# Mictronics/multi-sdr-gps-sim

Measured on NVIDIA H100. Metric: IQ Msamples/s, higher is better.
Workload: dtype f64 NCO / int32 accumulate / int8 out

## Files before the change

### include/gpsb200.h

```cpp
#ifndef GPSB200_H
#define GPSB200_H

#include <stdbool.h>
#include <stddef.h>
#include <stdint.h>

#ifdef __cplusplus
extern "C" {
#endif

#define GPSB200_SAMPLERATE        3000000
#define GPSB200_BLOCK_SAMPLES     300000
#define GPSB200_BLOCK_ELEMS       600000
#define GPSB200_MAX_CHAN          32
#define GPSB200_NAV_WORDS         60
#define GPSB200_CA_LEN            1023
#define GPSB200_SC08              1
#define GPSB200_SC16              2
#define GPSB200_HACKRF_BUFFER     262144

enum {
    GPSB200_OK = 0,
    GPSB200_ERR_ARG = -1,
    GPSB200_ERR_CUDA = -2,
// ... 63 lines not shown
    int32_t reset_inside[GPSB200_MAX_CHAN];
    double first_phase[GPSB200_MAX_CHAN];
    double value[GPSB200_MAX_CHAN];
} gpsb200_slice_link_t;
int gpsb200_slice_prepare(gpsb200_ctx_t *ctx, const gpsb200_chan_t *chans, int nblk, int nchan, int sample_size,
                          void *dst_device, void *dst_host, void *stream, gpsb200_slice_link_t *link);
int gpsb200_slice_wait(gpsb200_ctx_t *ctx);
int gpsb200_slice_probe(gpsb200_ctx_t *ctx, const int32_t *prn_in, const double *phase_guess_in, int eager);
int gpsb200_slice_finish(gpsb200_ctx_t *ctx, const int32_t *prn_in, const double *phase_in, int32_t *prn_out,
                         double *phase_out, gpsb200_stats_t *stats);
typedef void (*gpsb200_handoff_fn)(void *user, const int32_t *prn_out, const double *phase_out);
int gpsb200_slice_finish_cb(gpsb200_ctx_t *ctx, const int32_t *prn_in, const double *phase_in, int32_t *prn_out,
                            double *phase_out, gpsb200_stats_t *stats, gpsb200_handoff_fn handoff, void *user);
int gpsb200_slice_link_host(const gpsb200_chan_t *chans, int nblk, int nchan, gpsb200_slice_link_t *link);
int gpsb200_link_apply(const gpsb200_slice_link_t *link, int nchan, const int32_t *prn_in, const double *phase_in,
                       int32_t *prn_out, double *phase_out);

int gpsb200_debug_corrupt_chain(gpsb200_ctx_t *ctx, int on);

int gpsb200_debug_run_checkpoints(gpsb200_ctx_t *ctx, int nblk, int nchan, void *out);

int gpsb200_debug_block_probes(gpsb200_ctx_t *ctx, int nblk, int nchan, void *probes_out, double *seg_out,
                               double *guess_out);

int gpsb200_debug_synth_shape(gpsb200_ctx_t *ctx, int nblk, int nchan, int sample_size, const char **kernel,
                              int *ctas_per_block, int *runs_per_cta);

const char *gpsb200_synth_kernel_name(const gpsb200_ctx_t *ctx, int nchan);

int gpsb200_replay_device(gpsb200_ctx_t *ctx, void *dst_device, void *stream, int kernel_mask);

double gpsb200_carrier_advance(double carr_phase, double f_carr, int64_t nsamples);

int gpsb200_carrier_chain(const gpsb200_chan_t *chans, int nblk, int nchan, const double *phase_in,
                          double *phase_out, int threads);

int gpsb200_carrier_chain_device(gpsb200_ctx_t *ctx, const gpsb200_chan_t *chans, int nblk, int nchan,
                                 const double *phase_in, double *phase_out);

int gpsb200_carrier_probe_fixup(double start, double guess, double f_carr, int64_t nsamples, double *end_out);

int gpsb200_span_chain_host(const double *f_carr, int nblk, double start_true, double start_guess, double *starts_out);

int gpsb200_checkpoint_segments_host(double start_true, double start_guess, double f_carr, int run_samples,
                                     double *starts_out, int *nseg_out);

int gpsb200_carrier_probe_host(double guess, double f_carr, int64_t nsamples, int run_samples, int mode, void *probe_out,
                               double *seg_out);

int gpsb200_lanes_model_block(const gpsb200_chan_t *chans, int nchan, const uint32_t *nav, int run_samples, int force,
                              int16_t *iq, double *carr_out, int64_t *counters, uint32_t *signs);

int gpsb200_lanes_window_band_host(const uint32_t *steps, const uint32_t *bases, int64_t n, uint8_t *out);

int gpsb200_codegen(int prn, uint8_t ca[GPSB200_CA_LEN]);

#define GPSB200_ACQ_MAX_MS    100
#define GPSB200_ACQ_MAX_BINS  1024
#define GPSB200_ACQ_CODE_SAMPLES 3000
typedef struct gpsb200_acq_config {
    int64_t s0;
    int32_t ms;
    int32_t nprn;
    int32_t prn[32];
    double f_lo_hz;
    double step_hz;
    int32_t nbins;
    int32_t reserved;
} gpsb200_acq_config_t;
typedef struct gpsb200_acq_result {
    int32_t prn;
    int32_t bin;
    int32_t delay;
    int32_t reserved;
    double doppler_hz;
    double delay_chips;
    uint64_t p1, p2;
    double ratio;
} gpsb200_acq_result_t;
int gpsb200_acquire(gpsb200_ctx_t *ctx, const void *iq, int64_t nsamples, int sample_size, const gpsb200_acq_config_t *cfg,
                    gpsb200_acq_result_t *res, uint64_t *grid);
int gpsb200_acquire_device(gpsb200_ctx_t *ctx, const void *iq_device, int64_t nsamples, int sample_size,
                           const gpsb200_acq_config_t *cfg, gpsb200_acq_result_t *res, uint64_t *grid, void *stream);
int gpsb200_acquire_windows(gpsb200_ctx_t *ctx, const void *iq, int64_t nsamples, int sample_size,
                            const gpsb200_acq_config_t *cfg, const double *f_lo_prn, gpsb200_acq_result_t *res,
                            uint64_t *grid);
int gpsb200_debug_acq_split(gpsb200_ctx_t *ctx, int force, int nprn, int nbins);
int gpsb200_acquire_windows_device(gpsb200_ctx_t *ctx, const void *iq_device, int64_t nsamples, int sample_size,
                                   const gpsb200_acq_config_t *cfg, const double *f_lo_prn, gpsb200_acq_result_t *res,
                                   uint64_t *grid, void *stream);

#define GPSB200_TRK_CODE_STEP_NOM 1464583848u
#define GPSB200_TRK_CODE_STEP_MIN 1464095816u
#define GPSB200_TRK_CODE_STEP_MAX 1465072205u
#define GPSB200_TRK_FLL_EPOCHS    200
#define GPSB200_TRK_MAX_CHAN      32
typedef struct gpsb200_track_state {
    int32_t prn;
    int32_t epochs;
    int64_t sample;
    uint64_t code_phase;
    int64_t carr_freq;
    uint32_t carr_phase;
    int32_t carr_step;
    uint32_t code_step;
    int32_t prev_i, prev_q;
// ... 427 lines not shown
```

### multi-sdr-gps-sim_b200/__init__.py

```python
from .api import (
    BLOCK_ELEMS, BLOCK_SAMPLES, SC08, SC16, Chan, Config, Context, GpsB200Error, Stats,
    bind_numa, carrier_advance, span_chain_host, lanes_model_block, lanes_window_band, link_apply, slice_link_host, SliceLink, carrier_chain, codegen, scenario, lib, lib_path, CHAN_DTYPE,
    ScenarioConfig, LiveScenario, SteerState, parse_steer, KEYS, ERR_END, almanac_read, ALMANAC_RECORD_DTYPE, checkpoint_segments_host, RUN_CKPT_DTYPE,
    carrier_probe_host, CARRIER_PROBE_DTYPE, AcqConfig, ACQ_RESULT_DTYPE, ACQ_CODE_SAMPLES, acq_window_samples,
    TRACK_STATE_DTYPE, TRACK_EPOCH_DTYPE, NAV_BIT_DTYPE, NAV_WORD_DTYPE, NAV_SYNC_DTYPE, track_start, nav_decode, nav_word_check,
    nav_parity, EPHEMERIS_DTYPE, IONO_DTYPE, PVT_CHAN_DTYPE, PVT_CONFIG_DTYPE, FIX_DTYPE, FIX_OK, FIX_FEW,
    FIX_NO_CONVERGENCE, PVT_MAX_ITER, nav_words_of_frame, nav_ephemeris, nav_time_anchor, pvt_config,
    RAIM_CONFIG_DTYPE, RAIM_DTYPE, RAIM_PASS, RAIM_EXCLUDED, RAIM_ALERT, RAIM_UNAVAILABLE, RAIM_MAX_DOF,
    RAIM_MAX_EXCLUDE, raim_config, raim_thresholds, ARAIM_CONFIG_DTYPE, ARAIM_DTYPE, araim_config, araim_kfa,
    COARSE_CONFIG_DTYPE, COARSE_DTYPE, FIX_AMBIGUOUS, coarse_config, rinex_ephemeris,
    SEARCH_CONFIG_DTYPE, SEARCH_DTYPE, SEARCH_NODES, search_config, search_nodes,
    SKY_DTYPE, nav_almanac, almanac_predict,
    SNAPSHOT_CONFIG_DTYPE, SNAPSHOT_DTYPE, SNAP_OK, SNAP_WEAK, SNAP_NO_CONVERGENCE, SNAP_ITERATIONS, SNAP_MAX_ITER,
    snapshot_config, SNAP_BATCH_SCRATCH, snapshot_batch_pass,
    COLLECTIVE_CONFIG_DTYPE, COLLECTIVE_DTYPE, CD_SCORE_DTYPE, CD_CELL_DTYPE, CD_OK, CD_FEW, CD_AMBIGUOUS, CD_MAX_HYP,
    CD_MIN_USED, CD_Q_SHIFT, CD_Q_CAP, CD_AMBIGUOUS_PCT, collective_config,
)
from .synthetic import synthetic_chans
from . import sharding
```

### multi-sdr-gps-sim_b200/api.py

```python
import ctypes as C
import os

import numpy as np

BLOCK_SAMPLES = 300000
BLOCK_ELEMS = 600000
SC08, SC16 = 1, 2

_HERE = os.path.dirname(os.path.abspath(__file__))


def lib_path():
    return os.path.join(_HERE, "libgpsb200.so")


class GpsB200Error(RuntimeError):
    def __init__(self, code, msg):
        super().__init__("gpsb200 error %d: %s" % (code, msg))
        self.code = code


class Chan(C.Structure):
    _fields_ = [("prn", C.c_int32), ("iword", C.c_int32), ("ibit", C.c_int32), ("icode", C.c_int32),
                ("nav_frame", C.c_int32), ("reserved", C.c_int32),
# ... 320 lines not shown
    if rc:
        raise GpsB200Error(rc, "gpsb200_nav_almanac")
    return rec, int(wna.value)


SKY_DTYPE = np.dtype([("prn", "<i4"), ("valid", "<i4"), ("el_deg", "<f8"), ("az_deg", "<f8"), ("range_m", "<f8"),
                      ("doppler_hz", "<f8")])
assert SKY_DTYPE.itemsize == 40


def almanac_predict(rec, week, sow, x_a):
    r = np.ascontiguousarray(rec, dtype=ALMANAC_RECORD_DTYPE)
    assert r.size == 32
    x = np.ascontiguousarray(x_a, dtype=np.float64).reshape(3)
    out = np.zeros(32, SKY_DTYPE)
    rc = lib().gpsb200_almanac_predict(r.ctypes.data, int(week), float(sow), x.ctypes.data, out.ctypes.data)
    if rc:
        raise GpsB200Error(rc, "gpsb200_almanac_predict")
    return out


def nav_time_anchor(words, sync):
    w = np.ascontiguousarray(words, dtype=NAV_WORD_DTYPE)
    sy = np.array(sync, dtype=NAV_SYNC_DTYPE).reshape(1)
    ep, ms = C.c_int32(0), C.c_int64(0)
    rc = lib().gpsb200_nav_time_anchor(w.ctypes.data if w.size else None, w.size, sy.ctypes.data, C.byref(ep), C.byref(ms))
    if rc:
        raise GpsB200Error(rc, "gpsb200_nav_time_anchor")
    return int(ep.value), int(ms.value)


def pvt_config(s0, step, nfix, iono=None):
    c = np.zeros(1, PVT_CONFIG_DTYPE)[0]
    c["s0"], c["step"], c["nfix"] = int(s0), int(step), int(nfix)
    if iono is not None:
        c["iono"] = 1
        c["alpha"], c["beta"] = np.asarray(iono[0], np.float64), np.asarray(iono[1], np.float64)
    return c


HANDOFF_FN = C.CFUNCTYPE(None, C.c_void_p, C.POINTER(C.c_int32), C.POINTER(C.c_double))

_lib = None

EXPORTS = ["gpsb200_create", "gpsb200_destroy", "gpsb200_last_error", "gpsb200_version", "gpsb200_set_nav",
           "gpsb200_synth_blocks", "gpsb200_synth_blocks_scatter", "gpsb200_synth_blocks_device", "gpsb200_replay_device",
           "gpsb200_carrier_advance", "gpsb200_carrier_chain", "gpsb200_carrier_chain_device", "gpsb200_carrier_probe_fixup",
           "gpsb200_codegen", "gpsb200_acquire", "gpsb200_acquire_device", "gpsb200_acquire_windows",
           "gpsb200_acquire_windows_device", "gpsb200_debug_acq_split", "gpsb200_nav_almanac", "gpsb200_almanac_predict", "gpsb200_track_start",
           "gpsb200_track",
           "gpsb200_track_device", "gpsb200_nav_decode", "gpsb200_nav_word_check", "gpsb200_nav_parity",
           "gpsb200_nav_ephemeris", "gpsb200_nav_time_anchor", "gpsb200_pvt", "gpsb200_pvt_replay",
           "gpsb200_pvt_raim", "gpsb200_raim_thresholds", "gpsb200_pvt_araim", "gpsb200_araim_kfa", "gpsb200_pvt_coarse", "gpsb200_pvt_search", "gpsb200_search_nodes", "gpsb200_snapshot_measure", "gpsb200_snapshot_measure_device", "gpsb200_snapshot_batch", "gpsb200_snapshot_batch_device", "gpsb200_pvt_snapshot", "gpsb200_pvt_snapshot_search", "gpsb200_collective", "gpsb200_collective_device", "gpsb200_rinex_ephemeris", "gpsb200_bind_numa", "gpsb200_span_chain_host", "gpsb200_lanes_model_block",
           "gpsb200_lanes_window_band_host", "gpsb200_slice_prepare", "gpsb200_slice_probe",
           "gpsb200_slice_finish", "gpsb200_slice_finish_cb", "gpsb200_slice_wait", "gpsb200_link_apply", "gpsb200_slice_link_host", "gpsb200_debug_corrupt_chain", "gpsb200_synth_kernel_name",
           "gpsb200_debug_run_checkpoints", "gpsb200_checkpoint_segments_host",
           "gpsb200_carrier_probe_host", "gpsb200_debug_block_probes", "gpsb200_debug_synth_shape",
           "gpsb200_scenario_create", "gpsb200_scenario_destroy", "gpsb200_scenario_error",
           "gpsb200_scenario_blocks", "gpsb200_scenario_channels", "gpsb200_scenario_nav_frames",
           "gpsb200_scenario_chans", "gpsb200_scenario_nav", "gpsb200_scenario_almanac_date", "gpsb200_almanac_read",
           "gpsb200_scenario_open", "gpsb200_scenario_advance", "gpsb200_scenario_frame", "gpsb200_scenario_key",
           "gpsb200_scenario_steer_state", "gpsb200_scenario_open_now", "gpsb200_scenario_create_now",
           "gpsb200_scenario_start_date", "gpsb200_scenario_start_time",
           "fifo_create", "fifo_destroy", "fifo_wait_next", "fifo_wait_full", "fifo_halt", "fifo_acquire",
           "fifo_enqueue", "fifo_dequeue", "fifo_release", "fifo_set_compat_drop",
           "gpsb200_iqfile_start", "gpsb200_iqfile_stop", "gpsb200_fifo_push", "gpsb200_fifo_push_flush"]


def lib():
    global _lib
    if _lib is None:
        if not os.path.exists(lib_path()):
            raise GpsB200Error(-2, "libgpsb200.so not built (run __graft_entry__.build()); there is no CPU fallback")
        L = C.CDLL(lib_path())
        L.gpsb200_create.argtypes = [C.POINTER(Config), C.POINTER(C.c_void_p)]
        L.gpsb200_destroy.argtypes = [C.c_void_p]
        L.gpsb200_last_error.argtypes = [C.c_void_p]
        L.gpsb200_last_error.restype = C.c_char_p
        L.gpsb200_version.restype = C.c_char_p
        L.gpsb200_set_nav.argtypes = [C.c_void_p, C.c_int, C.c_int, C.c_void_p]
        L.gpsb200_synth_blocks.argtypes = [C.c_void_p, C.c_void_p, C.c_int, C.c_int, C.c_int, C.c_void_p,
                                           C.c_void_p, C.POINTER(Stats)]
        L.gpsb200_synth_blocks_scatter.argtypes = [C.c_void_p, C.c_void_p, C.c_int, C.c_int, C.c_int, C.c_void_p,
                                                   C.c_void_p, C.POINTER(Stats)]
        L.gpsb200_synth_blocks_device.argtypes = [C.c_void_p, C.c_void_p, C.c_int, C.c_int, C.c_int, C.c_void_p,
                                                  C.c_void_p, C.c_void_p, C.POINTER(Stats)]
        L.gpsb200_replay_device.argtypes = [C.c_void_p, C.c_void_p, C.c_void_p, C.c_int]
        L.gpsb200_carrier_advance.argtypes = [C.c_double, C.c_double, C.c_int64]
        L.gpsb200_carrier_advance.restype = C.c_double
        L.gpsb200_codegen.argtypes = [C.c_int, C.c_void_p]
        L.gpsb200_scenario_create.argtypes = [C.POINTER(ScenarioConfig), C.POINTER(C.c_void_p)]
        L.gpsb200_scenario_destroy.argtypes = [C.c_void_p]
        L.gpsb200_scenario_error.argtypes = [C.c_void_p]
        L.gpsb200_scenario_error.restype = C.c_char_p
        for fn in ("blocks", "channels", "nav_frames"):
            getattr(L, "gpsb200_scenario_" + fn).argtypes = [C.c_void_p]
        L.gpsb200_scenario_chans.argtypes = [C.c_void_p]
        L.gpsb200_scenario_chans.restype = C.c_void_p
        L.gpsb200_scenario_nav.argtypes = [C.c_void_p]
        L.gpsb200_scenario_nav.restype = C.c_void_p
        L.gpsb200_scenario_almanac_date.argtypes = [C.c_void_p]
        L.gpsb200_scenario_almanac_date.restype = C.c_char_p
        L.gpsb200_almanac_read.argtypes = [C.c_char_p, C.c_void_p, C.POINTER(C.c_int32)]
        L.gpsb200_scenario_open.argtypes = [C.POINTER(ScenarioConfig), C.POINTER(C.c_void_p)]
        L.gpsb200_scenario_open_now.argtypes = [C.POINTER(ScenarioConfig), C.POINTER(C.c_void_p)]
        L.gpsb200_scenario_create_now.argtypes = [C.POINTER(ScenarioConfig), C.POINTER(C.c_void_p)]
        L.gpsb200_scenario_start_date.argtypes = [C.c_void_p]
# ... 91 lines not shown
    ca = np.zeros(1023, np.uint8)
    rc = lib().gpsb200_codegen(prn, ca.ctypes.data)
    if rc:
        raise GpsB200Error(rc, "gpsb200_codegen(%d)" % prn)
    return ca


def carrier_advance(phase, f_carr, nsamples):
    return lib().gpsb200_carrier_advance(float(phase), float(f_carr), int(nsamples))


def carrier_chain(chans, phase_in=None, threads=16):
    a = np.ascontiguousarray(chans, dtype=CHAN_DTYPE)
    nblk, nchan = a.shape
    out = np.zeros(nchan, np.float64)
    pin = None if phase_in is None else np.ascontiguousarray(phase_in, dtype=np.float64)
    rc = lib().gpsb200_carrier_chain(a.ctypes.data, nblk, nchan, None if pin is None else pin.ctypes.data,
                                     out.ctypes.data, threads)
    if rc:
        raise GpsB200Error(rc, "gpsb200_carrier_chain")
    return out


def lanes_model_block(chans_row, nav_frame, run_samples=2400, force=0, want_signs=False):
    a = np.ascontiguousarray(chans_row, dtype=CHAN_DTYPE)
    nv = np.ascontiguousarray(nav_frame, dtype=np.uint32)
    iq = np.zeros(BLOCK_ELEMS, np.int16)
    co = np.zeros(a.size, np.float64)
    cnt = np.zeros(4, np.int64)
    signs = np.zeros((a.size, BLOCK_SAMPLES // 96, 3), np.uint32) if want_signs else None
    L = lib()
    L.gpsb200_lanes_model_block.argtypes = [C.c_void_p, C.c_int, C.c_void_p, C.c_int, C.c_int, C.c_void_p, C.c_void_p, C.c_void_p,
                                            C.c_void_p]
    rc = L.gpsb200_lanes_model_block(a.ctypes.data, a.size, nv.ctypes.data, run_samples, force, iq.ctypes.data, co.ctypes.data,
                                     cnt.ctypes.data, None if signs is None else signs.ctypes.data)
    if rc:
        raise GpsB200Error(rc, "gpsb200_lanes_model_block")
    return (iq, co, cnt, signs) if want_signs else (iq, co, cnt)


def lanes_window_band(steps, bases):
    st, bs = np.broadcast_arrays(np.asarray(steps, np.uint32), np.asarray(bases, np.uint32))
    st = np.ascontiguousarray(st.ravel())
    bs = np.ascontiguousarray(bs.ravel())
    out = np.zeros(st.size, np.uint8)
    L = lib()
    L.gpsb200_lanes_window_band_host.argtypes = [C.c_void_p, C.c_void_p, C.c_int64, C.c_void_p]
    rc = L.gpsb200_lanes_window_band_host(st.ctypes.data, bs.ctypes.data, st.size, out.ctypes.data)
    if rc:
        raise GpsB200Error(rc, "gpsb200_lanes_window_band_host")
    return out.astype(bool)


def span_chain_host(f_carr, start_true, start_guess):
    f = np.ascontiguousarray(f_carr, dtype=np.float64)
    out = np.zeros(f.size + 1)
    rc = lib().gpsb200_span_chain_host(f.ctypes.data, f.size, float(start_true), float(start_guess), out.ctypes.data)
    if rc < 0:
        raise GpsB200Error(rc, "gpsb200_span_chain_host")
    return out if rc == 1 else None


def checkpoint_segments_host(start_true, start_guess, f_carr, run_samples=2400):
    out = np.zeros(8)
    nseg = C.c_int(0)
    rc = lib().gpsb200_checkpoint_segments_host(float(start_true), float(start_guess), float(f_carr), int(run_samples),
                                            out.ctypes.data, C.byref(nseg))
    if rc < 0:
        raise GpsB200Error(rc, "gpsb200_checkpoint_segments_host")
    return rc == 1, out[:nseg.value]


def carrier_probe_host(guess, f_carr, nsamples=BLOCK_SAMPLES, run_samples=2400, mode=1):
    probe = np.zeros(1, CARRIER_PROBE_DTYPE)
    seg = np.zeros((2, 7))
    rc = lib().gpsb200_carrier_probe_host(float(guess), float(f_carr), int(nsamples), int(run_samples), int(mode),
                                          probe.ctypes.data, seg.ctypes.data)
    if rc:
        raise GpsB200Error(rc, "gpsb200_carrier_probe_host")
    return probe[0], seg


def slice_link_host(chans):
    a = np.ascontiguousarray(chans, dtype=CHAN_DTYPE)
    link = SliceLink()
    rc = lib().gpsb200_slice_link_host(a.ctypes.data, a.shape[0], a.shape[1], C.byref(link))
    if rc:
        raise GpsB200Error(rc, "gpsb200_slice_link_host")
    return link


def link_apply(link, nchan, prn_in=None, phase_in=None):
    pi = None if prn_in is None else np.ascontiguousarray(prn_in, dtype=np.int32)
    xi = None if phase_in is None else np.ascontiguousarray(phase_in, dtype=np.float64)
    po, xo = np.zeros(nchan, np.int32), np.zeros(nchan, np.float64)
    rc = lib().gpsb200_link_apply(C.byref(link), nchan, None if pi is None else pi.ctypes.data,
                                  None if xi is None else xi.ctypes.data, po.ctypes.data, xo.ctypes.data)
    if rc:
        raise GpsB200Error(rc, "gpsb200_link_apply")
    return po, xo


def almanac_read(path):
    rec = np.zeros(32, ALMANAC_RECORD_DTYPE)
    valid = C.c_int32(0)
    rc = lib().gpsb200_almanac_read(os.fsencode(path), rec.ctypes.data, C.byref(valid))
# ... 549 lines not shown
```

### multi-sdr-gps-sim_b200/csrc/synth_kernels.h

```cpp
#pragma once
#include <cuda_runtime.h>
#include <stdint.h>

namespace gpsb200 {

constexpr int kBlockSamples = 300000;
constexpr int kNavWords = 60;
constexpr int kChipWords = 33;
constexpr int kAtabRows = 513;

struct BlockChanDev {
    double c_carr;
    double c_code;
    double gain;
    double carr_in;
    double code0;
    int32_t prn;
    uint32_t nav0;
    int32_t frame;
    int32_t pad[3];
};
static_assert(sizeof(BlockChanDev) == 64, "BlockChanDev layout");

struct RunCkpt {
    double x;
    double y;
    uint32_t nav;
    uint32_t pad;
};
static_assert(sizeof(RunCkpt) == 24, "RunCkpt layout");

struct CarrierProbe;
struct SpanBlockState;

struct SpanRes {
    double start;
    double shift;
    int32_t variant;
    int32_t mode;
};
static_assert(sizeof(SpanRes) == 24, "SpanRes layout");

struct SynthArgs {
    const BlockChanDev *bc;
    const double *carr0;
    const double *guess;
    CarrierProbe *probe;
    CarrierProbe *probe_host;
    double *seg;
    CarrierProbe *span_sum;
    SpanBlockState *spec;
    const SpanRes *span_res;
    int span_blocks, nspan;
    RunCkpt *ck;
    const uint32_t *nav;
    int nav_stride;
    const uint32_t *chipbits;
    int32_t *atab;
    double *carr_end;
    double *last_end_host;
    int *chain_errors;
    void *out;
    int nblk, nchan, nruns, run_samples, runs_per_cta, ctas_per_block, iq16;
    int lanes;
};

cudaError_t launch_tables(const SynthArgs &a, cudaStream_t s);
cudaError_t launch_probe(const SynthArgs &a, cudaStream_t s);
cudaError_t launch_chain(const SynthArgs &a, cudaStream_t s);
cudaError_t launch_checkpoints(const SynthArgs &a, cudaStream_t s);
cudaError_t launch_synth(const SynthArgs &a, cudaStream_t s);
bool synth_lanes_applicable(const SynthArgs &a);
cudaError_t launch_synth_lanes(const SynthArgs &a, cudaStream_t s);
void synth_lanes_launch_shape(const SynthArgs &a, int *ctas, int *threads, size_t *smem, int *ctas_per_block,
                              int *runs_per_cta);
void synth_launch_shape(const SynthArgs &a, int *ctas, int *threads, size_t *smem, int *ctas_per_block, int *runs_per_cta);

}
```

### multi-sdr-gps-sim_b200/csrc/synth_lanes.cu

```cuda
#include <cuda_runtime.h>
#include <stdint.h>

#include "nco_exact.h"
#include "synth_kernels.h"
#include "synth_lanes.h"

namespace gpsb200 {

namespace {

constexpr int kLaneWarps = 16;
constexpr int kLaneCtas = 2;
constexpr int kLaneChipWords = 36;

struct LaneWin {
    uint32_t s0, s1, s2;
    uint32_t base;
};

struct LaneSteps {
    uint64_t D96, E96;
    uint32_t inv32, e22;
};

template <int CH>
struct LanesSmem {
    static constexpr int kWins = 32 / CH;
    uint32_t chips[CH][kLaneChipWords];
    uint32_t nav[CH][kNavWords];
    alignas(16) LaneWin win[kLaneWarps][kWins][CH];
    alignas(16) uint32_t step[CH];
    LaneSteps steps[CH];
    alignas(16) uint32_t stage[kLaneWarps][kWins * lanes::kWindow];
    uint32_t band[CH][lanes::kBandList + 1];
};
template <int CH>
constexpr size_t lanes_smem_bytes() { return sizeof(LanesSmem<CH>) + (size_t) CH * 2048; }

template <int OFF>
__device__ __forceinline__ int table_at(uint32_t p, uint32_t ta) {
    int e;
    asm volatile("{\n\t.reg .b32 i, ad;\n\tshr.b32 i, %1, 23;\n\tmad.lo.u32 ad, i, 4, %2;\n\tld.shared.b32 %0, [ad+%3];\n\t}"
                 : "=r"(e)
                 : "r"(p), "r"(ta), "n"(OFF));
    return e;
}

template <class ChipFn, class NavFn>
__device__ __noinline__ uint3 exact_signs_call(lanes::Anchor an, int w, ChipFn chips, NavFn nav) {
    uint32_t W[3];
    lanes::exact_signs(an, w, chips, nav, W);
    return make_uint3(W[0], W[1], W[2]);
}

__device__ __noinline__ int exact_index_call(lanes::Anchor an, int w, int n) {
    const uint64_t D = lanes::carr_step_fix(an.c);
    const uint64_t P = lanes::carr_fix(an.x0) + (uint64_t) w * ((uint64_t) lanes::kWindow * D);
    return lanes::exact_index(P, D, an, w, n);
}

__device__ __forceinline__ void add_if(int &acc, uint32_t w, uint32_t bit, int e) {
    asm("{\n\t.reg .pred p;\n\t.reg .b32 t;\n\tand.b32 t, %1, %2;\n\tsetp.ne.u32 p, t, 0;\n\t@p add.s32 %0, %0, %3;\n\t}"
        : "+r"(acc)
        : "r"(w), "r"(bit), "r"(e));
}

template <int NC>
__device__ __forceinline__ void window_sums(const LaneWin *wp, const uint32_t *sp, uint32_t ta, int nchan, uint32_t n0,
                                            uint32_t sbit, int accs[3]) {
    const int nc = NC > 0 ? NC : nchan;
    const uint32_t n1 = n0 + 32u, n2 = n0 + 64u;
    int all0 = 0, all1 = 0, all2 = 0, neg0 = 0, neg1 = 0, neg2 = 0;
#pragma unroll 4
    for (int c = 0; c < nc; c += 2, wp += 2, sp += 2, ta += 2 * 2048u) {
        const uint4 wa = *reinterpret_cast<const uint4 *>(&wp[0]);
        const uint4 wb = *reinterpret_cast<const uint4 *>(&wp[1]);
        const uint2 st = *reinterpret_cast<const uint2 *>(sp);
        const uint32_t a0 = wa.w + n0 * st.x, a1 = wa.w + n1 * st.x, a2 = wa.w + n2 * st.x;
        const uint32_t b0 = wb.w + n0 * st.y, b1 = wb.w + n1 * st.y, b2 = wb.w + n2 * st.y;
        const int ea0 = table_at<0>(a0, ta), eb0 = table_at<2048>(b0, ta);
        const int ea1 = table_at<0>(a1, ta), eb1 = table_at<2048>(b1, ta);
        const int ea2 = table_at<0>(a2, ta), eb2 = table_at<2048>(b2, ta);
        all0 += ea0 + eb0;
        all1 += ea1 + eb1;
        all2 += ea2 + eb2;
        add_if(neg0, wa.x, sbit, ea0);
        add_if(neg0, wb.x, sbit, eb0);
        add_if(neg1, wa.y, sbit, ea1);
        add_if(neg1, wb.y, sbit, eb1);
        add_if(neg2, wa.z, sbit, ea2);
        add_if(neg2, wb.z, sbit, eb2);
    }
    accs[0] = (int) ((uint32_t) all0 - 2u * (uint32_t) neg0);
    accs[1] = (int) ((uint32_t) all1 - 2u * (uint32_t) neg1);
    accs[2] = (int) ((uint32_t) all2 - 2u * (uint32_t) neg2);
}

template <bool IQ16, int CH>
__global__ void __launch_bounds__(kLaneWarps * 32, kLaneCtas) k_synth_lanes(SynthArgs a) {
    constexpr int WINS = 32 / CH;
    constexpr int SWZ = 32 / CH;
    constexpr int BYTES = IQ16 ? 4 : 2;
    extern __shared__ __align__(16) unsigned char smem_raw[];
    int32_t *tab = reinterpret_cast<int32_t *>(smem_raw);
    LanesSmem<CH> &sm = *reinterpret_cast<LanesSmem<CH> *>(smem_raw + CH * 2048);
    const uint32_t tab_base = (uint32_t) __cvta_generic_to_shared(smem_raw);
    constexpr uint32_t kFull = 0xFFFFFFFFu;

    const int b = blockIdx.x / a.ctas_per_block;
    const int g = blockIdx.x - b * a.ctas_per_block;
    const int tid = threadIdx.x, nthr = blockDim.x;
    const int lane = tid & 31, warp = tid >> 5;
    const int nchan = a.nchan;
    const BlockChanDev *bc = a.bc + (size_t) b * nchan;

    {
        const int32_t *src = a.atab + (size_t) b * kAtabRows * 32;
        for (int i = tid; i < 512 * CH; i += nthr) {
            const int k = i / CH, c = i - k * CH;
            tab[c * 512 + ((k + c * SWZ) & 511)] = c < nchan ? src[k * 32 + c] : 0;
        }
        for (int i = tid; i < CH * kLaneChipWords; i += nthr) {
            const int c = i / kLaneChipWords, w = i - c * kLaneChipWords;
            uint32_t v = 0;
            if (c < nchan && bc[c].prn > 0) {
                const uint32_t *cw = a.chipbits + bc[c].prn * kChipWords;
                v = w < kChipWords ? cw[w] : __funnelshift_r(cw[w - 32], cw[w - 31], 1);
            }
            sm.chips[c][w] = v;
        }
        for (int i = tid; i < CH * kNavWords; i += nthr) {
            const int c = i / kNavWords, w = i - c * kNavWords;
            uint32_t v = 0;
            if (c < nchan && bc[c].prn > 0) v = a.nav[((size_t) bc[c].frame * a.nav_stride + c) * kNavWords + w];
            sm.nav[c][w] = v;
        }
        if (warp == kLaneWarps - 1 && lane < CH) {
            const bool ok = lane < nchan && bc[lane].prn > 0;
            lanes::ChanRun k;
            lanes::init_steps(k, ok, ok ? bc[lane].c_carr : 0.0, ok ? bc[lane].c_code : 0.0);
            sm.steps[lane] = LaneSteps{k.D96, k.E96, k.inv32, k.e22};
            sm.step[lane] = lanes::fast_step(k);
            lanes::band_residues(lanes::fast_step(k), &sm.band[lane][0]);
        }
    }
    __syncthreads();

    const int ch = lane & (CH - 1), half = lane / CH;
    const bool chan_ok = ch < nchan && bc[ch < nchan ? ch : 0].prn > 0;
    const uint32_t *nav_row = &sm.nav[ch][0];
    const uint32_t *chip_row = &sm.chips[ch][0];
    const uint32_t *band_row = &sm.band[ch][0];
    auto navf = [nav_row](int iw) { return nav_row[iw]; };
    auto chipf = [chip_row](int i) { return chip_row[i]; };
    const uint32_t n0 = (uint32_t) lane, n1 = n0 + 32u, n2 = n0 + 64u;
    const uint32_t sbit = 1u << lanes::sign_pos(lane);
    const int nwin = a.run_samples / lanes::kWindow;
    uint32_t *stage = &sm.stage[warp][0];

    const int run_first = g * a.runs_per_cta;
    const int run_last = min(run_first + a.runs_per_cta, a.nruns);
#pragma unroll 1
    for (int r = run_first + warp; r < run_last; r += kLaneWarps) {
        auto anchor = [&](int c) {
            const RunCkpt k0 = a.ck[((size_t) b * a.nruns + r) * nchan + c];
            return lanes::Anchor{k0.x, k0.y, bc[c].c_carr, bc[c].c_code, k0.nav};
        };
        lanes::ChanRun s;
        auto load_steps = [&]() {
            const LaneSteps k = sm.steps[ch];
            s.D96 = k.D96;
            s.E96 = k.E96;
            s.inv32 = k.inv32;
            s.e22 = k.e22;
        };
        {
            const lanes::Anchor an = chan_ok ? anchor(ch) : lanes::Anchor{0.0, 0.0, 0.0, 0.0, 0u};
            lanes::init_run(s, chan_ok, an.x0, an.y0, an.navpos, an.c, an.d, navf);
        }
        if (WINS == 2 && chan_ok && half == 1) {
            load_steps();
            lanes::advance_window(s, navf);
        }
        uint4 *dst = reinterpret_cast<uint4 *>(reinterpret_cast<char *>(a.out) +
                                               ((size_t) b * kBlockSamples + (size_t) r * a.run_samples) * BYTES);

#pragma unroll 1
        for (int w = 0; w < nwin; w += WINS) {
            uint32_t flagged;
            {
                uint32_t S[3] = {0u, 0u, 0u};
                uint32_t base = (uint32_t) (ch * SWZ) << 23;
                bool band = false;
                if (chan_ok) load_steps();
                if (chan_ok && w > 0) {
#pragma unroll
                    for (int i = 0; i < WINS; i++) lanes::advance_window(s, navf);
                }
                if (chan_ok && w + half < nwin) {
                    base += lanes::fast_base(s);
                    band = lanes::window_band_risky(band_row, base);
                    if (!lanes::window_signs(s, chipf, navf, S)) {
                        const uint3 e = exact_signs_call(anchor(ch), w + half, chipf, navf);
                        S[0] = e.x;
                        S[1] = e.y;
                        S[2] = e.z;
                    }
                }
                *reinterpret_cast<uint4 *>(&sm.win[warp][half][ch]) = make_uint4(S[0], S[1], S[2], base);
                flagged = __ballot_sync(kFull, band);
            }
            __syncwarp();

#pragma unroll
// ... 11 lines not shown
                    const uint32_t st = sm.step[c];
                    const uint32_t p0 = wv.w + n0 * st, p1 = wv.w + n1 * st, p2 = wv.w + n2 * st;
                    const bool risky = lanes::fast_risky(p0) | lanes::fast_risky(p1) | lanes::fast_risky(p2);
                    if (!risky) continue;
                    const lanes::Anchor ac = anchor(c);
                    const uint32_t ps[3] = {p0, p1, p2}, sw[3] = {wv.x, wv.y, wv.z};
#pragma unroll
                    for (int j = 0; j < 3; j++) {
                        if (!lanes::fast_risky(ps[j])) continue;
                        const int kf = (int) (ps[j] >> 23);
                        const int k = exact_index_call(ac, w + hh, 32 * j + lane);
                        const int fix = tab[c * 512 + ((k + c * SWZ) & 511)] - tab[c * 512 + kf];
                        accs[j] += (sw[j] & sbit) ? -fix : fix;
                    }
                }
#pragma unroll
                for (int j = 0; j < 3; j++) {
                    const uint32_t p = (uint32_t) accs[j];
                    const uint32_t x = p + ((p & 0x8000u) << 1);
                    const int n = hh * lanes::kWindow + 32 * j + lane;
                    if (IQ16)
                        stage[n] = x;
                    else
                        reinterpret_cast<uint16_t *>(stage)[n] = (uint16_t) (((p >> 4) & 0xFFu) | ((x >> 12) & 0xFF00u));
                }
            }
            __syncwarp();
            {
                constexpr int kVec = WINS * lanes::kWindow * BYTES / 16;
                const int nvec = WINS == 1 || nwin - w >= WINS ? kVec : kVec / WINS;
                const uint4 *srcv = reinterpret_cast<const uint4 *>(stage);
#pragma unroll
                for (int i = lane; i < ((kVec + 31) & ~31); i += 32)
                    if (i < nvec) dst[i] = srcv[i];
                dst += kVec;
            }
        }
    }
}

}

bool synth_lanes_applicable(const SynthArgs &a) {
    return a.lanes && a.nchan <= 32 && a.run_samples % lanes::kWindow == 0 && a.run_samples <= lanes::kMaxRun;
}

static int device_sms() {
    int dev = 0, n = 0;
    if (cudaGetDevice(&dev) != cudaSuccess || cudaDeviceGetAttribute(&n, cudaDevAttrMultiProcessorCount, dev) != cudaSuccess)
        return 132;
    return n;
}

static void lanes_shape(const SynthArgs &a, int *ctas_per_block, int *runs_per_cta) {
    int per_block = (40 * kLaneCtas * device_sms() + a.nblk - 1) / a.nblk;
    if (per_block > 16) per_block = 16;
    if (per_block < 1) per_block = 1;
    int per_cta = (a.nruns + per_block - 1) / per_block;
    per_cta = (per_cta + kLaneWarps - 1) / kLaneWarps * kLaneWarps;
    per_block = (a.nruns + per_cta - 1) / per_cta;
    *ctas_per_block = per_block;
    *runs_per_cta = per_cta;
}

template <bool IQ16, int CH>
static cudaError_t launch_lanes_t(const SynthArgs &a, cudaStream_t s) {
    const size_t smem = lanes_smem_bytes<CH>();
    cudaError_t e = cudaFuncSetAttribute(k_synth_lanes<IQ16, CH>, cudaFuncAttributeMaxDynamicSharedMemorySize, (int) smem);
    if (e != cudaSuccess) return e;
    k_synth_lanes<IQ16, CH><<<a.nblk * a.ctas_per_block, kLaneWarps * 32, smem, s>>>(a);
    return cudaGetLastError();
}

cudaError_t launch_synth_lanes(const SynthArgs &a_in, cudaStream_t s) {
    SynthArgs a = a_in;
    lanes_shape(a, &a.ctas_per_block, &a.runs_per_cta);
    if (a.nchan <= 16) return a.iq16 ? launch_lanes_t<true, 16>(a, s) : launch_lanes_t<false, 16>(a, s);
    return a.iq16 ? launch_lanes_t<true, 32>(a, s) : launch_lanes_t<false, 32>(a, s);
}

void synth_lanes_launch_shape(const SynthArgs &a, int *ctas, int *threads, size_t *smem, int *ctas_per_block,
                              int *runs_per_cta) {
    int per_block, per_cta;
    lanes_shape(a, &per_block, &per_cta);
    *ctas = a.nblk * per_block;
    *threads = kLaneWarps * 32;
    *smem = a.nchan <= 16 ? lanes_smem_bytes<16>() : lanes_smem_bytes<32>();
    *ctas_per_block = per_block;
    *runs_per_cta = per_cta;
}

}
```

### multi-sdr-gps-sim_b200/csrc/synth_lanes.h

```cpp
#pragma once
#include <stdint.h>

#include "nco_exact.h"

namespace gpsb200 {
namespace lanes {

constexpr int kWindow = 96;
constexpr int kMaxRun = 2400;
constexpr uint64_t kOne54 = 1ull << 54;
constexpr uint64_t kCodeWrap54 = 1023ull << 54;
constexpr uint64_t kBandCode = 1ull << 22;
constexpr uint64_t kBandCarr = 1ull << 23;
constexpr uint32_t kBandFast = 128;

GPSB_HD bool code_step_ok(double c_code) { return c_code >= 0.33855 && c_code < 0.34340; }

GPSB_HD uint64_t carr_fix(double x) { return (x >= 0.0 && x < 1.0) ? (uint64_t) (x * 0x1p64) : 0; }
GPSB_HD uint64_t carr_step_fix(double c) {
    const double a = c < 0.0 ? -c : c;
    const uint64_t m = (uint64_t) (a * 0x1p64);
    return c < 0.0 ? (uint64_t) 0 - m : m;
}
GPSB_HD uint64_t code_fix(double y) { return (uint64_t) (y * 0x1p54); }
// ... 210 lines not shown
constexpr int kBandList = 128;
constexpr uint32_t kBandPad = kMod23;

GPSB_HD int band_distinct(uint32_t u) {
    if (u == 0) return 1;
    const uint32_t period = kMod23 / (u & (0u - u));
    return period < (uint32_t) kWindow ? (int) period : kWindow;
}

GPSB_HD void band_residues(uint32_t step, uint32_t *R) {
    const uint32_t u = step & (kMod23 - 1);
    const int m = band_distinct(u);
    int a = 0, b = 0;
    uint32_t ra = kMod23, rb = 0;
    for (int n = 1; n < m; n++) {
        const uint32_t r = ((uint32_t) n * u) & (kMod23 - 1);
        if (r < ra) ra = r, a = n;
        if (r > rb) rb = r, b = n;
    }
    const uint32_t db = kMod23 - rb;
    int n = 0;
    uint32_t r = 0;
    for (int k = 0; k < m; k++) {
        R[k] = r;
        if (n + a < m) {
            n += a;
            r += ra;
        } else if (n >= b) {
            n -= b;
            r += db;
        } else {
            n += a - b;
            r += ra + db;
        }
    }
    for (int k = m; k < kBandList; k++) R[k] = kBandPad;
}

GPSB_HD bool window_band_risky(const uint32_t *R, uint32_t base) {
    const uint32_t t = (0u - kBandFast - base) & (kMod23 - 1);
    const uint32_t te = t + kBandFast;
    uint32_t i = 0, lo = 0;
#pragma unroll
    for (uint32_t s = kBandList / 2; s > 0; s >>= 1) {
        const uint32_t v = R[i + s - 1];
        if (v < te) {
            i += s;
            lo = v;
        }
    }
    return lo >= t;
}

}
}
```

Baseline: 71420.

## Give whole blocks to early CTAs and batch table-fill loads into registers

Changes the launch mapping so that, for many blocks with 32 channels, the first waves of CTAs each process an entire block's runs. Only the last two waves split blocks across CTAs. This amortizes the per-CTA shared-memory table prologue over more runs while keeping the tail balanced. The prologue is also moved into a noinline function that issues all global loads (vectorized int4 for the amplitude table) into registers before any shared stores, to overlap load latency. The cost is a more complex CTA-to-run mapping and higher register use in the prologue.

```diff
diff --git a/include/gpsb200.h b/include/gpsb200.h
--- a/include/gpsb200.h
+++ b/include/gpsb200.h
@@ -139,6 +139,8 @@
                               int16_t *iq, double *carr_out, int64_t *counters, uint32_t *signs);
 
 int gpsb200_lanes_window_band_host(const uint32_t *steps, const uint32_t *bases, int64_t n, uint8_t *out);
+
+int gpsb200_lanes_launch_map_host(int nblk, int nruns, int sms, int nchan, int *shape, int *map);
 
 int gpsb200_codegen(int prn, uint8_t ca[GPSB200_CA_LEN]);
 
diff --git a/multi-sdr-gps-sim_b200/__init__.py b/multi-sdr-gps-sim_b200/__init__.py
--- a/multi-sdr-gps-sim_b200/__init__.py
+++ b/multi-sdr-gps-sim_b200/__init__.py
@@ -1,6 +1,6 @@
 from .api import (
     BLOCK_ELEMS, BLOCK_SAMPLES, SC08, SC16, Chan, Config, Context, GpsB200Error, Stats,
-    bind_numa, carrier_advance, span_chain_host, lanes_model_block, lanes_window_band, link_apply, slice_link_host, SliceLink, carrier_chain, codegen, scenario, lib, lib_path, CHAN_DTYPE,
+    bind_numa, carrier_advance, span_chain_host, lanes_model_block, lanes_window_band, lanes_launch_map, link_apply, slice_link_host, SliceLink, carrier_chain, codegen, scenario, lib, lib_path, CHAN_DTYPE,
     ScenarioConfig, LiveScenario, SteerState, parse_steer, KEYS, ERR_END, almanac_read, ALMANAC_RECORD_DTYPE, checkpoint_segments_host, RUN_CKPT_DTYPE,
     carrier_probe_host, CARRIER_PROBE_DTYPE, AcqConfig, ACQ_RESULT_DTYPE, ACQ_CODE_SAMPLES, acq_window_samples,
     TRACK_STATE_DTYPE, TRACK_EPOCH_DTYPE, NAV_BIT_DTYPE, NAV_WORD_DTYPE, NAV_SYNC_DTYPE, track_start, nav_decode, nav_word_check,
diff --git a/multi-sdr-gps-sim_b200/api.py b/multi-sdr-gps-sim_b200/api.py
--- a/multi-sdr-gps-sim_b200/api.py
+++ b/multi-sdr-gps-sim_b200/api.py
@@ -396,7 +396,7 @@
            "gpsb200_track_device", "gpsb200_nav_decode", "gpsb200_nav_word_check", "gpsb200_nav_parity",
            "gpsb200_nav_ephemeris", "gpsb200_nav_time_anchor", "gpsb200_pvt", "gpsb200_pvt_replay",
            "gpsb200_pvt_raim", "gpsb200_raim_thresholds", "gpsb200_pvt_araim", "gpsb200_araim_kfa", "gpsb200_pvt_coarse", "gpsb200_pvt_search", "gpsb200_search_nodes", "gpsb200_snapshot_measure", "gpsb200_snapshot_measure_device", "gpsb200_snapshot_batch", "gpsb200_snapshot_batch_device", "gpsb200_pvt_snapshot", "gpsb200_pvt_snapshot_search", "gpsb200_collective", "gpsb200_collective_device", "gpsb200_rinex_ephemeris", "gpsb200_bind_numa", "gpsb200_span_chain_host", "gpsb200_lanes_model_block",
-           "gpsb200_lanes_window_band_host", "gpsb200_slice_prepare", "gpsb200_slice_probe",
+           "gpsb200_lanes_window_band_host", "gpsb200_lanes_launch_map_host", "gpsb200_slice_prepare", "gpsb200_slice_probe",
            "gpsb200_slice_finish", "gpsb200_slice_finish_cb", "gpsb200_slice_wait", "gpsb200_link_apply", "gpsb200_slice_link_host", "gpsb200_debug_corrupt_chain", "gpsb200_synth_kernel_name",
            "gpsb200_debug_run_checkpoints", "gpsb200_checkpoint_segments_host",
            "gpsb200_carrier_probe_host", "gpsb200_debug_block_probes", "gpsb200_debug_synth_shape",
@@ -594,6 +594,19 @@
     return out.astype(bool)
 
 
+def lanes_launch_map(nblk, nruns, sms, nchan=32):
+    shape = np.zeros(5, np.int32)
+    L = lib()
+    L.gpsb200_lanes_launch_map_host.argtypes = [C.c_int, C.c_int, C.c_int, C.c_int, C.c_void_p, C.c_void_p]
+    rc = L.gpsb200_lanes_launch_map_host(int(nblk), int(nruns), int(sms), int(nchan), shape.ctypes.data, None)
+    if rc:
+        raise GpsB200Error(rc, "gpsb200_lanes_launch_map_host")
+    m = np.zeros((int(shape[3]), 3), np.int32)
+    L.gpsb200_lanes_launch_map_host(int(nblk), int(nruns), int(sms), int(nchan), shape.ctypes.data, m.ctypes.data)
+    keys = ("whole", "per_block", "per_cta", "ctas", "warps")
+    return {k: int(v) for k, v in zip(keys, shape)}, m
+
+
 def span_chain_host(f_carr, start_true, start_guess):
     f = np.ascontiguousarray(f_carr, dtype=np.float64)
     out = np.zeros(f.size + 1)
diff --git a/multi-sdr-gps-sim_b200/csrc/synth_kernels.h b/multi-sdr-gps-sim_b200/csrc/synth_kernels.h
--- a/multi-sdr-gps-sim_b200/csrc/synth_kernels.h
+++ b/multi-sdr-gps-sim_b200/csrc/synth_kernels.h
@@ -62,6 +62,7 @@
     int *chain_errors;
     void *out;
     int nblk, nchan, nruns, run_samples, runs_per_cta, ctas_per_block, iq16;
+    int whole_blocks;
     int lanes;
 };
 
diff --git a/multi-sdr-gps-sim_b200/csrc/synth_lanes.cu b/multi-sdr-gps-sim_b200/csrc/synth_lanes.cu
--- a/multi-sdr-gps-sim_b200/csrc/synth_lanes.cu
+++ b/multi-sdr-gps-sim_b200/csrc/synth_lanes.cu
@@ -1,6 +1,8 @@
 #include <cuda_runtime.h>
 #include <stdint.h>
-
+#include <stdlib.h>
+
+#include "../../include/gpsb200.h"
 #include "nco_exact.h"
 #include "synth_kernels.h"
 #include "synth_lanes.h"
@@ -12,6 +14,10 @@
 constexpr int kLaneWarps = 16;
 constexpr int kLaneCtas = 2;
 constexpr int kLaneChipWords = 36;
+
+#ifndef GPSB200_LANES_PROLOGUE_REPS
+#define GPSB200_LANES_PROLOGUE_REPS 1
+#endif
 
 struct LaneWin {
     uint32_t s0, s1, s2;
@@ -96,6 +102,65 @@
     accs[2] = (int) ((uint32_t) all2 - 2u * (uint32_t) neg2);
 }
 
+template <int CH>
+__device__ __noinline__ void fill_tables(const int32_t *src, const BlockChanDev *bc, const uint32_t *chipbits,
+                                         const uint32_t *nav, int nav_stride, int nchan, int32_t *tab,
+                                         uint32_t (*chips)[kLaneChipWords], uint32_t (*navw)[kNavWords]) {
+    constexpr int SWZ = 32 / CH;
+    constexpr uint32_t kFull = 0xFFFFFFFFu;
+    const int tid = threadIdx.x, lane = tid & 31;
+    constexpr int kThr = kLaneWarps * 32;
+    constexpr int kTabVec = 512 * CH / 4 / kThr;
+    constexpr int kChipPer = (CH * kLaneChipWords + kThr - 1) / kThr;
+    constexpr int kNavPer = (CH * kNavWords + kThr - 1) / kThr;
+    const bool own = lane < nchan;
+    const int own_prn = own ? bc[lane].prn : 0, own_frame = own ? bc[lane].frame : 0;
+    int4 tv[kTabVec];
+#pragma unroll
+    for (int j = 0; j < kTabVec; j++) {
+        const int q = tid + j * kThr, k = q / (CH / 4), c0 = (q - k * (CH / 4)) * 4;
+        tv[j] = c0 < nchan ? *reinterpret_cast<const int4 *>(src + k * 32 + c0) : make_int4(0, 0, 0, 0);
+    }
+    uint32_t cv[kChipPer], nv[kNavPer];
+#pragma unroll
+    for (int j = 0; j < kChipPer; j++) {
+        const int i = tid + j * kThr, c = min(i / kLaneChipWords, CH - 1), w = i - c * kLaneChipWords;
+        const int prn = __shfl_sync(kFull, own_prn, c);
+        cv[j] = 0;
+        if (i < CH * kLaneChipWords && c < nchan && prn > 0) {
+            const uint32_t *cw = chipbits + prn * kChipWords;
+            cv[j] = w < kChipWords ? cw[w] : __funnelshift_r(cw[w - 32], cw[w - 31], 1);
+        }
+    }
+#pragma unroll
+    for (int j = 0; j < kNavPer; j++) {
+        const int i = tid + j * kThr, c = min(i / kNavWords, CH - 1), w = i - c * kNavWords;
+        const int prn = __shfl_sync(kFull, own_prn, c), frame = __shfl_sync(kFull, own_frame, c);
+        nv[j] = 0;
+        if (i < CH * kNavWords && c < nchan && prn > 0) nv[j] = nav[((size_t) frame * nav_stride + c) * kNavWords + w];
+    }
+#pragma unroll
+    for (int j = 0; j < kTabVec; j++) {
+        const int q = tid + j * kThr, k = q / (CH / 4), c0 = (q - k * (CH / 4)) * 4;
+        const int e[4] = {tv[j].x, tv[j].y, tv[j].z, tv[j].w};
+#pragma unroll
+        for (int m = 0; m < 4; m++) {
+            const int c = c0 + m;
+            tab[c * 512 + ((k + c * SWZ) & 511)] = c < nchan ? e[m] : 0;
+        }
+    }
+#pragma unroll
+    for (int j = 0; j < kChipPer; j++) {
+        const int i = tid + j * kThr;
+        if (i < CH * kLaneChipWords) (&chips[0][0])[i] = cv[j];
+    }
+#pragma unroll
+    for (int j = 0; j < kNavPer; j++) {
+        const int i = tid + j * kThr;
+        if (i < CH * kNavWords) (&navw[0][0])[i] = nv[j];
+    }
+}
+
 template <bool IQ16, int CH>
 __global__ void __launch_bounds__(kLaneWarps * 32, kLaneCtas) k_synth_lanes(SynthArgs a) {
     constexpr int WINS = 32 / CH;
@@ -107,34 +172,18 @@
     const uint32_t tab_base = (uint32_t) __cvta_generic_to_shared(smem_raw);
     constexpr uint32_t kFull = 0xFFFFFFFFu;
 
-    const int b = blockIdx.x / a.ctas_per_block;
-    const int g = blockIdx.x - b * a.ctas_per_block;
-    const int tid = threadIdx.x, nthr = blockDim.x;
+    int b, run_first, run_last;
+    lanes::cta_runs(lanes::LaunchShape{a.whole_blocks, a.ctas_per_block, a.runs_per_cta}, a.nruns, (int) blockIdx.x, &b,
+                    &run_first, &run_last);
+    const int tid = threadIdx.x;
     const int lane = tid & 31, warp = tid >> 5;
     const int nchan = a.nchan;
     const BlockChanDev *bc = a.bc + (size_t) b * nchan;
 
-    {
-        const int32_t *src = a.atab + (size_t) b * kAtabRows * 32;
-        for (int i = tid; i < 512 * CH; i += nthr) {
-            const int k = i / CH, c = i - k * CH;
-            tab[c * 512 + ((k + c * SWZ) & 511)] = c < nchan ? src[k * 32 + c] : 0;
-        }
-        for (int i = tid; i < CH * kLaneChipWords; i += nthr) {
-            const int c = i / kLaneChipWords, w = i - c * kLaneChipWords;
-            uint32_t v = 0;
-            if (c < nchan && bc[c].prn > 0) {
-                const uint32_t *cw = a.chipbits + bc[c].prn * kChipWords;
-                v = w < kChipWords ? cw[w] : __funnelshift_r(cw[w - 32], cw[w - 31], 1);
-            }
-            sm.chips[c][w] = v;
-        }
-        for (int i = tid; i < CH * kNavWords; i += nthr) {
-            const int c = i / kNavWords, w = i - c * kNavWords;
-            uint32_t v = 0;
-            if (c < nchan && bc[c].prn > 0) v = a.nav[((size_t) bc[c].frame * a.nav_stride + c) * kNavWords + w];
-            sm.nav[c][w] = v;
-        }
+#pragma unroll 1
+    for (int rep = 0; rep < GPSB200_LANES_PROLOGUE_REPS; rep++) {
+        fill_tables<CH>(a.atab + (size_t) b * kAtabRows * 32, bc, a.chipbits, a.nav, a.nav_stride, nchan, tab, sm.chips,
+                        sm.nav);
         if (warp == kLaneWarps - 1 && lane < CH) {
             const bool ok = lane < nchan && bc[lane].prn > 0;
             lanes::ChanRun k;
@@ -143,8 +192,8 @@
             sm.step[lane] = lanes::fast_step(k);
             lanes::band_residues(lanes::fast_step(k), &sm.band[lane][0]);
         }
-    }
-    __syncthreads();
+        __syncthreads();
+    }
 
     const int ch = lane & (CH - 1), half = lane / CH;
     const bool chan_ok = ch < nchan && bc[ch < nchan ? ch : 0].prn > 0;
@@ -158,8 +207,6 @@
     const int nwin = a.run_samples / lanes::kWindow;
     uint32_t *stage = &sm.stage[warp][0];
 
-    const int run_first = g * a.runs_per_cta;
-    const int run_last = min(run_first + a.runs_per_cta, a.nruns);
 #pragma unroll 1
     for (int r = run_first + warp; r < run_last; r += kLaneWarps) {
         auto anchor = [&](int c) {
@@ -277,15 +324,15 @@
     return n;
 }
 
-static void lanes_shape(const SynthArgs &a, int *ctas_per_block, int *runs_per_cta) {
-    int per_block = (40 * kLaneCtas * device_sms() + a.nblk - 1) / a.nblk;
-    if (per_block > 16) per_block = 16;
-    if (per_block < 1) per_block = 1;
-    int per_cta = (a.nruns + per_block - 1) / per_block;
-    per_cta = (per_cta + kLaneWarps - 1) / kLaneWarps * kLaneWarps;
-    per_block = (a.nruns + per_cta - 1) / per_cta;
-    *ctas_per_block = per_block;
-    *runs_per_cta = per_cta;
+static lanes::LaunchShape lanes_shape(const SynthArgs &a) {
+    const char *ev = getenv("GPSB200_LANES_CTAS");
+    const int forced = ev ? atoi(ev) : 0;
+    if (forced > 0) {
+        int per_cta = (a.nruns + forced - 1) / forced;
+        per_cta = (per_cta + kLaneWarps - 1) / kLaneWarps * kLaneWarps;
+        return lanes::LaunchShape{0, (a.nruns + per_cta - 1) / per_cta, per_cta};
+    }
+    return lanes::launch_shape(a.nblk, a.nruns, kLaneCtas * device_sms(), kLaneWarps, a.nchan > 16);
 }
 
 template <bool IQ16, int CH>
@@ -293,26 +340,44 @@
     const size_t smem = lanes_smem_bytes<CH>();
     cudaError_t e = cudaFuncSetAttribute(k_synth_lanes<IQ16, CH>, cudaFuncAttributeMaxDynamicSharedMemorySize, (int) smem);
     if (e != cudaSuccess) return e;
-    k_synth_lanes<IQ16, CH><<<a.nblk * a.ctas_per_block, kLaneWarps * 32, smem, s>>>(a);
+    const lanes::LaunchShape sh{a.whole_blocks, a.ctas_per_block, a.runs_per_cta};
+    k_synth_lanes<IQ16, CH><<<lanes::launch_ctas(sh, a.nblk), kLaneWarps * 32, smem, s>>>(a);
     return cudaGetLastError();
 }
 
 cudaError_t launch_synth_lanes(const SynthArgs &a_in, cudaStream_t s) {
     SynthArgs a = a_in;
-    lanes_shape(a, &a.ctas_per_block, &a.runs_per_cta);
+    const lanes::LaunchShape sh = lanes_shape(a);
+    a.whole_blocks = sh.whole;
+    a.ctas_per_block = sh.per_block;
+    a.runs_per_cta = sh.per_cta;
     if (a.nchan <= 16) return a.iq16 ? launch_lanes_t<true, 16>(a, s) : launch_lanes_t<false, 16>(a, s);
     return a.iq16 ? launch_lanes_t<true, 32>(a, s) : launch_lanes_t<false, 32>(a, s);
 }
 
 void synth_lanes_launch_shape(const SynthArgs &a, int *ctas, int *threads, size_t *smem, int *ctas_per_block,
                               int *runs_per_cta) {
-    int per_block, per_cta;
-    lanes_shape(a, &per_block, &per_cta);
-    *ctas = a.nblk * per_block;
+    const lanes::LaunchShape sh = lanes_shape(a);
+    *ctas = lanes::launch_ctas(sh, a.nblk);
     *threads = kLaneWarps * 32;
     *smem = a.nchan <= 16 ? lanes_smem_bytes<16>() : lanes_smem_bytes<32>();
-    *ctas_per_block = per_block;
-    *runs_per_cta = per_cta;
-}
-
-}
+    *ctas_per_block = sh.per_block;
+    *runs_per_cta = sh.per_cta;
+}
+
+}
+
+extern "C" int gpsb200_lanes_launch_map_host(int nblk, int nruns, int sms, int nchan, int *shape, int *map) {
+    using namespace gpsb200;
+    if (nblk < 1 || nruns < 1 || sms < 1 || nchan < 1 || nchan > 32 || !shape) return GPSB200_ERR_ARG;
+    const lanes::LaunchShape sh = lanes::launch_shape(nblk, nruns, kLaneCtas * sms, kLaneWarps, nchan > 16);
+    const int ctas = lanes::launch_ctas(sh, nblk);
+    shape[0] = sh.whole;
+    shape[1] = sh.per_block;
+    shape[2] = sh.per_cta;
+    shape[3] = ctas;
+    shape[4] = kLaneWarps;
+    if (map)
+        for (int i = 0; i < ctas; i++) lanes::cta_runs(sh, nruns, i, &map[3 * i], &map[3 * i + 1], &map[3 * i + 2]);
+    return GPSB200_OK;
+}
diff --git a/multi-sdr-gps-sim_b200/csrc/synth_lanes.h b/multi-sdr-gps-sim_b200/csrc/synth_lanes.h
--- a/multi-sdr-gps-sim_b200/csrc/synth_lanes.h
+++ b/multi-sdr-gps-sim_b200/csrc/synth_lanes.h
@@ -286,5 +286,37 @@
     return lo >= t;
 }
 
-}
-}
+struct LaunchShape {
+    int whole;
+    int per_block;
+    int per_cta;
+};
+
+GPSB_HD LaunchShape launch_shape(int nblk, int nruns, int slots, int warps, bool whole) {
+    int per_block = (40 * slots + nblk - 1) / nblk;
+    if (per_block > 16) per_block = 16;
+    if (per_block < 1) per_block = 1;
+    int per_cta = (nruns + per_block - 1) / per_block;
+    per_cta = (per_cta + warps - 1) / warps * warps;
+    per_block = (nruns + per_cta - 1) / per_cta;
+    const int waves = (nblk + slots - 1) / slots;
+    return LaunchShape{whole && waves > 2 ? (waves - 2) * slots : 0, per_block, per_cta};
+}
+
+GPSB_HD void cta_runs(const LaunchShape &s, int nruns, int cta, int *blk, int *r0, int *r1) {
+    if (cta < s.whole) {
+        *blk = cta;
+        *r0 = 0;
+        *r1 = nruns;
+        return;
+    }
+    const int t = cta - s.whole, q = t / s.per_block, g = t - q * s.per_block;
+    *blk = s.whole + q;
+    *r0 = g * s.per_cta;
+    *r1 = *r0 + s.per_cta < nruns ? *r0 + s.per_cta : nruns;
+}
+
+GPSB_HD int launch_ctas(const LaunchShape &s, int nblk) { return s.whole + (nblk - s.whole) * s.per_block; }
+
+}
+}
```

New measurement: 72860, median of 6. 1.02x the previous value.
